# rafaelvp-db/databricks-distributed-deep-learning

Measured on AMD Instinct MI355X. Metric: ResNet-50 images/sec (whole node), higher is better.
Workload: dtype bf16

## Files before the change

### csrc/kernels/gemm_duo.hip

```cpp
#include "ddl_lds.h"

#include <cstdlib>

namespace {

constexpr int TM = 256, TN = 128, DBK = 32, NST = 3, NTH = 256;
constexpr int A_BYTES = TM * DBK * 2;
constexpr int B_BYTES = TN * DBK * 2;
constexpr int ST_BYTES = A_BYTES + B_BYTES;
constexpr int GROUP_M = 8;

enum { LKC = 0, LKO = 1, LCONV = 2 };
enum { E_BF16 = 0, E_GELU = 1, E_DGELU = 2, E_BNB = 3 };

struct DuoParams {
    const bf16_t* A;
    const bf16_t* B;
    long lda, ldb;
    bf16_t* C;
    long ldc;
    int M, N, K;
    const bf16_t* bias;
    const bf16_t* res;
    bf16_t* aux;
    float* colstats;
    int tiles_m, tiles_n;
    int cN, cH, cW, cC, cP, cQ, cstride, h_off, w_off, h_step, w_step, cR, cS;
    FastDiv fd_PQ, fd_Q, fd_C, fd_S;
    const uint8_t* bn_mask;
    const float* bn_mean;
    const float* bn_istd;
    int splits, kt_per_split;
    bf16_t* ws;
    int accumulate;
    const bf16_t* zero;
};

__device__ __forceinline__ bf16x8 frag_kc(const char* sub) {
    const int l = threadIdx.x & 63;
    return *reinterpret_cast<const bf16x8*>(sub + swz_kc((l & 15) * 64 + (l >> 4) * 16));
}
__device__ __attribute__((aligned(16))) uint4 g_duo_zero[1];

template <int LA, int LB, int EK>
__global__ __launch_bounds__(NTH, 2) void gemm_duo_k(DuoParams p) {
    __shared__ __attribute__((aligned(16))) char smem[NST * ST_BYTES];
    const int w = __builtin_amdgcn_readfirstlane(threadIdx.x >> 6), l = threadIdx.x & 63;
    const int wm = w >> 1, wn = w & 1;

    int tm, tn, split = 0;
    {
        const int nwg = p.tiles_m * p.tiles_n, n = nwg * p.splits, bid = blockIdx.x;
        const int xcd = bid & 7, qn = n >> 3, rn = n & 7;
        const int q = (xcd < rn ? xcd * (qn + 1) : rn * (qn + 1) + (xcd - rn) * qn) + (bid >> 3);
        split = q / nwg;
        const int wg = q - split * nwg;
        const int per_group = GROUP_M * p.tiles_n;
        const int grp = wg / per_group, first_m = grp * GROUP_M;
        const int gsz = min(p.tiles_m - first_m, GROUP_M);
        const int wl = wg - grp * per_group;
        tm = first_m + wl % gsz;
        tn = wl / gsz;
    }
    const int m0 = tm * TM, n0 = tn * TN;
    const int kbase = split * p.kt_per_split;
    const int nt = min(p.K / DBK - kbase, p.kt_per_split);

    const int lb = swz_kc(l * 16);
    const int r_in = lb >> 6, kcol = ((lb >> 4) & 3) * 8;
    const long a_bytes = LA == LCONV ? (long)p.cN * p.cH * p.cW * p.cC * 2
                       : (LA == LKO ? (long)p.K * p.lda * 2 : (long)p.M * p.lda * 2);
    const __amdgpu_buffer_rsrc_t ars_op =
        __builtin_amdgcn_make_buffer_rsrc(const_cast<bf16_t*>(p.A), 0, (int)a_bytes, 0x00020000);
    const __amdgpu_buffer_rsrc_t brs_op = __builtin_amdgcn_make_buffer_rsrc(
        const_cast<bf16_t*>(p.B), 0, (int)((long)(LB == LKC ? p.N : p.K) * p.ldb * 2), 0x00020000);
    int ao[4], bo[2];
    const bf16_t* abase[4];
    uint32_t vmask[4];
#pragma unroll
    for (int s = 0; s < 4; ++s) {
        const int m = m0 + (4 * w + s) * 16 + r_in;
        if (LA == LCONV) {
            const int mm = m < p.M ? m : 0;
            const int n = (int)fdiv((uint32_t)mm, p.fd_PQ);
            const int rem = mm - n * p.cP * p.cQ;
            const int pp = (int)fdiv((uint32_t)rem, p.fd_Q);
            const int qq = rem - pp * p.cQ;
            const int hb = pp * p.cstride + p.h_off, wb = qq * p.cstride + p.w_off;
            uint32_t mk = 0;
            if (m < p.M) {
                for (int rr = 0; rr < p.cR; ++rr)
                    for (int ss = 0; ss < p.cS; ++ss) {
                        const int hh = hb + rr * p.h_step, ww = wb + ss * p.w_step;
                        if ((unsigned)hh < (unsigned)p.cH && (unsigned)ww < (unsigned)p.cW) mk |= 1u << (rr * p.cS + ss);
                    }
            }
            vmask[s] = mk;
            abase[s] = p.A + ((long)(n * p.cH + hb) * p.cW + wb) * p.cC + kcol;
            ao[s] = 0;
        } else if (LA == LKO) {
            const int u = 4 * w + s, krow = (u & 7) * 4 + (l >> 4);
            ao[s] = (krow * (int)p.lda + m0 + (u >> 3) * 128 + 8 * ((l & 15) ^ swz_ko(krow))) * 2;
        } else {
            ao[s] = (min(m, p.M - 1) * (int)p.lda + kcol) * 2;
        }
    }
#pragma unroll
    for (int s = 0; s < 2; ++s) {
        if (LB == LKC) {
            bo[s] = ((n0 + (2 * w + s) * 16 + r_in) * (int)p.ldb + kcol) * 2;
        } else {
            const int krow = (2 * w + s) * 4 + (l >> 4);
            bo[s] = (krow * (int)p.ldb + n0 + 8 * ((l & 15) ^ swz_ko(krow))) * 2;
        }
    }
    const int b_kstep = LB == LKC ? DBK * 2 : DBK * (int)p.ldb * 2;
    auto stage = [&](int kt, int slot) {
        kt += kbase;
        char* sb = smem + slot * ST_BYTES;
        if constexpr (LA == LKO) {
#pragma unroll
            for (int s = 0; s < 4; ++s) {
                const int u = 4 * w + s;
                __builtin_amdgcn_raw_ptr_buffer_load_lds(ars_op, (lds_void*)(sb + (u >> 3) * 8192 + (u & 7) * 1024), 16,
                                                         ao[s], kt * DBK * (int)p.lda * 2, 0, 0);
            }
        } else if constexpr (LA == LCONV) {
            const int k0 = kt * DBK;
            const int tap = (int)fdiv((uint32_t)k0, p.fd_C), ci = k0 - tap * p.cC;
            const int rr = (int)fdiv((uint32_t)tap, p.fd_S), ss = tap - rr * p.cS;
            const long toff = (long)(rr * p.h_step * p.cW + ss * p.w_step) * p.cC + ci;
#pragma unroll
            for (int s = 0; s < 4; ++s) {
                const bool ok = (vmask[s] >> tap) & 1u;
                glds16(ok ? abase[s] + toff : p.zero, sb + (4 * w + s) * 1024);
            }
        } else {
#pragma unroll
            for (int s = 0; s < 4; ++s)
                __builtin_amdgcn_raw_ptr_buffer_load_lds(ars_op, (lds_void*)(sb + (4 * w + s) * 1024), 16, ao[s],
                                                         kt * (DBK * 2), 0, 0);
        }
#pragma unroll
        for (int s = 0; s < 2; ++s)
            __builtin_amdgcn_raw_ptr_buffer_load_lds(brs_op, (lds_void*)(sb + A_BYTES + (2 * w + s) * 1024), 16, bo[s],
                                                     kt * b_kstep, 0, 0);
    };

    f32x4 acc[8][4];
#pragma unroll
    for (int i = 0; i < 8; ++i)
#pragma unroll
        for (int j = 0; j < 4; ++j) acc[i][j] = (f32x4){0.f, 0.f, 0.f, 0.f};

    bf16x8 fa0[8], fb0[4], fa1[8], fb1[4];
    auto read_frags = [&](int slot, bf16x8 (&fa)[8], bf16x8 (&fb)[4]) {
        const char* sb = smem + slot * ST_BYTES;
        const int lane = threadIdx.x & 63;
#pragma unroll
        for (int j = 0; j < 4; ++j)
            fb[j] = LB == LKC ? frag_kc(sb + A_BYTES + (wn * 4 + j) * 1024) : frag_ko(sb + A_BYTES, wn * 64 + j * 16, lane);
#pragma unroll
        for (int i = 0; i < 8; ++i) fa[i] = LA == LKO ? frag_ko(sb + wm * 8192, i * 16, lane) : frag_kc(sb + (wm * 8 + i) * 1024);
// ... 33 lines not shown
        const int s1 = slot == 2 ? 0 : slot + 1;
        step(t, slot, fa0, fb0, fa1, fb1);
        step(t + 1, s1, fa1, fb1, fa0, fb0);
        slot = s1 == 2 ? 0 : s1 + 1;
    }
    if (t < nt) step(t, slot, fa0, fb0, fa1, fb1);

    const int r16 = l & 15, g4 = (l >> 4) * 4;
    const int mw = m0 + wm * 128;
    const int nw = n0 + wn * 64;
    const uint32_t cbytes = (uint32_t)((long)p.M * p.ldc * 2);
    float bv[4][4];
#pragma unroll
    for (int j = 0; j < 4; ++j) {
        if (EK != E_DGELU && p.bias) {
            const uint2 b2 = *reinterpret_cast<const uint2*>(p.bias + nw + j * 16 + g4);
            bv[j][0] = lo_f(b2.x); bv[j][1] = hi_f(b2.x); bv[j][2] = lo_f(b2.y); bv[j][3] = hi_f(b2.y);
        } else {
            bv[j][0] = bv[j][1] = bv[j][2] = bv[j][3] = 0.f;
        }
    }
    const bf16_t* pre = EK == E_BF16 ? p.res : (EK == E_DGELU ? (const bf16_t*)p.aux : nullptr);
    float bnm[4][4], bns[4][4];
    if (EK == E_BNB) {
#pragma unroll
        for (int j = 0; j < 4; ++j) {
            const f32x4 mv = *reinterpret_cast<const f32x4*>(p.bn_mean + nw + j * 16 + g4);
            const f32x4 sv = *reinterpret_cast<const f32x4*>(p.bn_istd + nw + j * 16 + g4);
#pragma unroll
            for (int e = 0; e < 4; ++e) { bnm[j][e] = mv[e]; bns[j][e] = sv[e]; }
        }
    }
    u32x2 rb[8][4];
    if (pre) {
        const __amdgpu_buffer_rsrc_t prs =
            __builtin_amdgcn_make_buffer_rsrc(const_cast<bf16_t*>(pre), 0, (int)cbytes, 0x00020000);
#pragma unroll
        for (int i = 0; i < 8; ++i)
#pragma unroll
            for (int j = 0; j < 4; ++j)
                rb[i][j] = __builtin_amdgcn_raw_buffer_load_b64(
                    prs, (int)(((long)(mw + i * 16 + r16) * p.ldc + nw + j * 16 + g4) * 2), 0, 0);
    }
    const int wr0 = wm * 128 + r16;
    auto img_off = [&](int i, int j) {
        const int u = (wn * 8 + j * 2 + (l >> 5)) * 2 + ((l >> 4) & 1);
        return (wr0 + i * 16) * 256 + ((u ^ r16) << 3);
    };
    BARRIER();
    const bool stats = EK != E_GELU && p.colstats;
    u32x2 yk[8][4];
    const __amdgpu_buffer_rsrc_t xrs =
        __builtin_amdgcn_make_buffer_rsrc(EK == E_BNB ? (void*)p.aux : (void*)p.C, 0, (int)cbytes, 0x00020000);
    const __amdgpu_buffer_rsrc_t rrs =
        __builtin_amdgcn_make_buffer_rsrc(EK == E_BNB && p.res ? (void*)p.res : (void*)p.C, 0, (int)cbytes, 0x00020000);
    const __amdgpu_buffer_rsrc_t mrs = __builtin_amdgcn_make_buffer_rsrc(
        EK == E_BNB && p.bn_mask ? (void*)p.bn_mask : (void*)p.C, 0, (int)(cbytes / 16), 0x00020000);
#pragma unroll
    for (int j = 0; j < 4; ++j) {
        float cs[4] = {0.f, 0.f, 0.f, 0.f}, cq[4] = {0.f, 0.f, 0.f, 0.f};
        u32x2 bx[8], br[8];
        uint32_t bmk[8];
        if (EK == E_BNB) {
#pragma unroll
            for (int i = 0; i < 8; ++i) {
                const int o = (mw + i * 16 + r16) * (int)p.ldc + nw + j * 16 + g4;
                bx[i] = __builtin_amdgcn_raw_buffer_load_b64(xrs, o * 2, 0, 0);
                br[i] = p.res ? __builtin_amdgcn_raw_buffer_load_b64(rrs, o * 2, 0, 0) : u32x2{0u, 0u};
                bmk[i] = p.bn_mask ? (uint32_t)__builtin_amdgcn_raw_buffer_load_b8(mrs, o >> 3, 0, 0) >> (o & 4) : 0xfu;
            }
        }
#pragma unroll
        for (int i = 0; i < 8; ++i) {
            const int m = mw + i * 16 + r16;
            const f32x4 a = acc[i][j];
            uint32_t lo, hi;
            if (EK == E_BF16) {
                float rv[4] = {0.f, 0.f, 0.f, 0.f};
                if (pre) { rv[0] = lo_f(rb[i][j][0]); rv[1] = hi_f(rb[i][j][0]); rv[2] = lo_f(rb[i][j][1]); rv[3] = hi_f(rb[i][j][1]); }
                lo = pack2bf(a[0] + bv[j][0] + rv[0], a[1] + bv[j][1] + rv[1]);
                hi = pack2bf(a[2] + bv[j][2] + rv[2], a[3] + bv[j][3] + rv[3]);
                *reinterpret_cast<uint2*>(smem + img_off(i, j)) = make_uint2(lo, hi);
            } else if (EK == E_GELU) {
                const float z[4] = {a[0] + bv[j][0], a[1] + bv[j][1], a[2] + bv[j][2], a[3] + bv[j][3]};
                const f32x2_t y0 = gelu_erf2(f32x2_t{z[0], z[1]}), y1 = gelu_erf2(f32x2_t{z[2], z[3]});
                lo = pack2bf(y0.x, y0.y);
                hi = pack2bf(y1.x, y1.y);
                yk[i][j] = u32x2{lo, hi};
                *reinterpret_cast<uint2*>(smem + img_off(i, j)) =
                    p.aux ? make_uint2(pack2bf(z[0], z[1]), pack2bf(z[2], z[3])) : make_uint2(lo, hi);
            } else if (EK == E_BNB) {
                float v[4];
#pragma unroll
                for (int e = 0; e < 4; ++e) {
                    const uint32_t rw = br[i][e >> 1];
                    const float rv = (e & 1) ? hi_f(rw) : lo_f(rw);
                    v[e] = ((bmk[i] >> e) & 1u) ? a[e] + rv : 0.f;
                }
                lo = pack2bf(v[0], v[1]);
                hi = pack2bf(v[2], v[3]);
                *reinterpret_cast<uint2*>(smem + img_off(i, j)) = make_uint2(lo, hi);
            } else {
                const u32x2 z2 = rb[i][j];
                const f32x2_t d0 = f32x2_t{a[0], a[1]} * gelu_erf_grad2(f32x2_t{lo_f(z2[0]), hi_f(z2[0])});
                const f32x2_t d1 = f32x2_t{a[2], a[3]} * gelu_erf_grad2(f32x2_t{lo_f(z2[1]), hi_f(z2[1])});
                lo = pack2bf(d0.x, d0.y);
                hi = pack2bf(d1.x, d1.y);
                *reinterpret_cast<uint2*>(smem + img_off(i, j)) = make_uint2(lo, hi);
            }
            if (stats) {
                const bool keep = m < p.M;
                const float tv[4] = {keep ? lo_f(lo) : 0.f, keep ? hi_f(lo) : 0.f, keep ? lo_f(hi) : 0.f,
                                     keep ? hi_f(hi) : 0.f};
                if (EK == E_BNB) {
                    const float xv[4] = {lo_f(bx[i][0]), hi_f(bx[i][0]), lo_f(bx[i][1]), hi_f(bx[i][1])};
#pragma unroll
                    for (int e = 0; e < 4; ++e) {
                        cs[e] += tv[e];
                        cq[e] += tv[e] * (xv[e] - bnm[j][e]) * bns[j][e];
                    }
                } else {
#pragma unroll
                    for (int e = 0; e < 4; ++e) {
                        cs[e] += tv[e];
                        cq[e] += tv[e] * tv[e];
                    }
                }
            }
        }
        if (stats) {
#pragma unroll
            for (int e = 0; e < 4; ++e) {
                cs[e] = row16_sum(cs[e]);
                cq[e] = row16_sum(cq[e]);
            }
            if (r16 == 0) {
                float* row = p.colstats + (long)(tm * 2 + wm) * 2 * p.N;
                const int n = nw + j * 16 + g4;
                *reinterpret_cast<f32x4*>(row + n) = (f32x4){cs[0], cs[1], cs[2], cs[3]};
                *reinterpret_cast<f32x4*>(row + p.N + n) = (f32x4){cq[0], cq[1], cq[2], cq[3]};
            }
        }
    }
    auto store_image = [&](bf16_t* dst, long ld, uint32_t bytes, bool acc_c, bool nt = false) {
        asm volatile("s_waitcnt lgkmcnt(0)" ::: "memory");
        BARRIER();
        const __amdgpu_buffer_rsrc_t rs = __builtin_amdgcn_make_buffer_rsrc(dst, 0, (int)bytes, 0x00020000);
        const int c = l & 15;
        const bool odd = (l >> 4) & 1;
#pragma unroll
        for (int it = 0; it < 16; ++it) {
            const int r = w * 64 + it * 4 + (l >> 4);
            u32x4 v = *reinterpret_cast<const u32x4*>(smem + r * 256 + ((c ^ ((r >> 1) & 7)) << 4));
            if (odd) v = u32x4{v[2], v[3], v[0], v[1]};
            const int off = (int)(((long)(m0 + r) * ld + n0 + c * 8) * 2);
            if (acc_c) {
                const u32x4 o = __builtin_amdgcn_raw_buffer_load_b128(rs, off, 0, 0);
#pragma unroll
                for (int e = 0; e < 4; ++e)
                    v[e] = pack2bf(lo_f(v[e]) + lo_f(o[e]), hi_f(v[e]) + hi_f(o[e]));
            }
            if (nt) __builtin_amdgcn_raw_buffer_store_b128(v, rs, off, 0, 2);
            else __builtin_amdgcn_raw_buffer_store_b128(v, rs, off, 0, 0);
        }
    };
    if (p.splits > 1) {
        store_image(p.ws + (long)split * p.M * p.N, p.N, (uint32_t)((long)p.M * p.N * 2), false);
        return;
    }
    if (EK == E_GELU && p.aux) {
        store_image(p.aux, p.ldc, cbytes, false, true);
        asm volatile("s_waitcnt lgkmcnt(0)" ::: "memory");
        BARRIER();
#pragma unroll
        for (int i = 0; i < 8; ++i)
#pragma unroll
            for (int j = 0; j < 4; ++j)
                *reinterpret_cast<uint2*>(smem + img_off(i, j)) = make_uint2(yk[i][j][0], yk[i][j][1]);
    }
    store_image(p.C, p.ldc, cbytes, p.accumulate != 0);
}

__global__ __launch_bounds__(256) void duo_reduce_k(const bf16_t* __restrict__ ws, bf16_t* __restrict__ C, long ldc,
                                                    int M, int N, int splits, int accumulate) {
    const long n8 = N / 8, total = (long)M * n8, slab = (long)M * N;
    for (long i = (long)blockIdx.x * blockDim.x + threadIdx.x; i < total; i += (long)gridDim.x * blockDim.x) {
        const int m = (int)(i / n8), n = (int)(i - (long)m * n8) * 8;
        float v[8] = {0.f, 0.f, 0.f, 0.f, 0.f, 0.f, 0.f, 0.f};
        const bf16_t* pb = ws + (long)m * N + n;
        auto add = [&](const uint4& r) {
            const uint32_t wd[4] = {r.x, r.y, r.z, r.w};
#pragma unroll
            for (int e = 0; e < 4; ++e) { v[2 * e] += lo_f(wd[e]); v[2 * e + 1] += hi_f(wd[e]); }
        };
        int s = 0;
        for (; s + 4 <= splits; s += 4) {
            uint4 r[4];
#pragma unroll
            for (int j = 0; j < 4; ++j) r[j] = *reinterpret_cast<const uint4*>(pb + (s + j) * slab);
#pragma unroll
            for (int j = 0; j < 4; ++j) add(r[j]);
        }
        for (; s < splits; ++s) add(*reinterpret_cast<const uint4*>(pb + s * slab));
        bf16_t* cp = C + (long)m * ldc + n;
        if (accumulate) {
            float o[8];
            load8(cp, o);
#pragma unroll
            for (int e = 0; e < 8; ++e) v[e] += o[e];
        }
        store8(cp, v);
    }
}

template <int LA, int LB>
int launch(const DuoParams& p, int ek, hipStream_t st) {
    const dim3 grid(p.tiles_m * p.tiles_n), block(NTH);
    switch (ek) {
        case E_BF16: hipLaunchKernelGGL((gemm_duo_k<LA, LB, E_BF16>), grid, block, 0, st, p); break;
        case E_GELU: hipLaunchKernelGGL((gemm_duo_k<LA, LB, E_GELU>), grid, block, 0, st, p); break;
        case E_DGELU: hipLaunchKernelGGL((gemm_duo_k<LA, LB, E_DGELU>), grid, block, 0, st, p); break;
        default: hipLaunchKernelGGL((gemm_duo_k<LA, LB, E_BNB>), grid, block, 0, st, p); break;
    }
    return (int)hipGetLastError();
}

}

DDL_API int ddl_gemm_duo(int mode, const void* A, long lda, const void* B, long ldb, void* C, long ldc, int M, int N,
                         int K, const void* bias, int act, void* aux, const void* res, float* colstats, const int* conv,
                         hipStream_t st) {
    BnbArgs bn{};
    if (act == 5) bn = ddl_take_bnb();
    if (M <= 0 || N <= 0) return 0;
    if (mode != 0 && mode != 1 && mode != 3) return -1;
    if (mode == 3 && (!conv || conv[3] % 32 || conv[13] != conv[4] || conv[14] != conv[5] || conv[15] != 1 ||
                      conv[16] != 0 || conv[17] != 0 || K != conv[11] * conv[12] * conv[3] ||
                      conv[11] * conv[12] > 32))
        return -1;
    if (N % TN || K % DBK || K <= 0 || lda % 8 || ldb % 8 || ldc % 8 || (mode != 3 && lda < K) || ldc < N ||
        (mode == 1 ? ldb < N : ldb < K) || ((uintptr_t)A & 15) || ((uintptr_t)B & 15) || ((uintptr_t)C & 15))
        return -1;
    int ek;
    if (act == 0) ek = E_BF16;
    else if (act == 1 && !res) ek = E_GELU;
    else if (act == 4 && aux && !bias && !res) ek = E_DGELU;
    else if (act == 5 && aux && !bias && colstats && bn.mean && bn.istd && ldc == N) ek = E_BNB;
    else return -2;
    if (ek == E_GELU && colstats) return -2;
    if ((res && ((uintptr_t)res & 7)) || (aux && ((uintptr_t)aux & 15)) || (bias && ((uintptr_t)bias & 7))) return -1;
    const long a_bytes = mode == 3 ? (long)conv[0] * conv[1] * conv[2] * conv[3] * 2 : (long)M * lda * 2;
    const long b_bytes = (long)(mode == 1 ? K : N) * ldb * 2, c_bytes = (long)M * ldc * 2;
    if (a_bytes >= (1L << 31) || b_bytes >= (1L << 31) || c_bytes >= (1L << 31)) return -1;
    DuoParams p{};
    p.A = (const bf16_t*)A; p.B = (const bf16_t*)B; p.lda = lda; p.ldb = ldb;
    p.C = (bf16_t*)C; p.ldc = ldc; p.M = M; p.N = N; p.K = K;
    p.bias = (const bf16_t*)bias; p.res = (const bf16_t*)res; p.aux = (bf16_t*)aux; p.colstats = colstats;
    p.bn_mask = bn.mask; p.bn_mean = bn.mean; p.bn_istd = bn.istd;
    p.splits = 1;
    p.kt_per_split = K / DBK;
    p.tiles_m = (M + TM - 1) / TM;
    p.tiles_n = N / TN;
    if (mode == 3) {
        static const bf16_t* zp[64] = {};
        int dev = 0;
        if (hipGetDevice(&dev) != hipSuccess || dev < 0 || dev >= 64) return -1;
        if (!zp[dev]) {
            void* a = nullptr;
            if (hipGetSymbolAddress(&a, HIP_SYMBOL(g_duo_zero)) != hipSuccess || !a) return -1;
            zp[dev] = (const bf16_t*)a;
        }
        p.zero = zp[dev];
        p.cN = conv[0]; p.cH = conv[1]; p.cW = conv[2]; p.cC = conv[3]; p.cP = conv[4]; p.cQ = conv[5];
        p.cstride = conv[6]; p.h_off = conv[7]; p.w_off = conv[8]; p.h_step = conv[9]; p.w_step = conv[10];
        p.cR = conv[11]; p.cS = conv[12];
        p.fd_PQ = make_fastdiv((uint32_t)(p.cP * p.cQ));
        p.fd_Q = make_fastdiv((uint32_t)p.cQ);
        p.fd_C = make_fastdiv((uint32_t)p.cC);
        p.fd_S = make_fastdiv((uint32_t)std::max(1, p.cS));
        return launch<LCONV, LKC>(p, ek, st);
    }
    return mode == 0 ? launch<LKC, LKC>(p, ek, st) : launch<LKC, LKO>(p, ek, st);
}

DDL_API int ddl_gemm_duo_tn(const void* A, long lda, const void* B, long ldb, void* C, long ldc, int M, int N, int K,
                            int splits, int accumulate, void* ws, long ws_elems, hipStream_t st) {
    if (M <= 0 || N <= 0) return 0;
    if (M % TM || N % TN || K % DBK || K <= 0 || lda % 8 || ldb % 8 || ldc % 8 || lda < M || ldb < N || ldc < N ||
        ((uintptr_t)A & 15) || ((uintptr_t)B & 15) || ((uintptr_t)C & 15))
        return -1;
    if ((long)K * lda * 2 >= (1L << 31) || (long)K * ldb * 2 >= (1L << 31) || (long)M * ldc * 2 >= (1L << 31)) return -1;
    const int nkt = K / DBK;
    if (splits < 1) splits = 1;
    if (splits > nkt) splits = nkt;
    DuoParams p{};
    p.A = (const bf16_t*)A; p.B = (const bf16_t*)B; p.lda = lda; p.ldb = ldb;
    p.C = (bf16_t*)C; p.ldc = ldc; p.M = M; p.N = N; p.K = K;
    p.tiles_m = M / TM;
    p.tiles_n = N / TN;
    p.kt_per_split = (nkt + splits - 1) / splits;
    splits = (nkt + p.kt_per_split - 1) / p.kt_per_split;
    p.splits = splits;
    p.accumulate = accumulate;
    if (splits > 1) {
        if (!ws || ws_elems < (long)splits * M * N || ((uintptr_t)ws & 15) || (long)splits * M * N * 2 >= (1L << 31))
            return -1;
        p.ws = (bf16_t*)ws;
    }
    const dim3 grid(p.tiles_m * p.tiles_n * splits);
    hipLaunchKernelGGL((gemm_duo_k<LKO, LKO, E_BF16>), grid, dim3(NTH), 0, st, p);
    if (splits > 1) {
        const long total = (long)M * (N / 8);
        const int g = (int)std::min<long>(16384, (total + 255) / 256);
        duo_reduce_k<<<g, 256, 0, st>>>(p.ws, p.C, ldc, M, N, splits, accumulate);
    }
    const int rc = (int)hipGetLastError();
    return rc ? -rc - 1 : splits;
}
```

### databricks_distributed_deep_learning_amd/ops/_lib.py

```python
from __future__ import annotations

import ctypes
import os
from typing import Optional

import torch

_PKG_DIR = os.path.dirname(os.path.dirname(os.path.abspath(__file__)))
LIB_PATH = os.environ.get("DDL_NATIVE_LIB") or os.path.join(_PKG_DIR, "_native", "libddl_kernels.so")

_lib: Optional[ctypes.CDLL] = None
_load_error: Optional[str] = None
_mode = os.environ.get("DDL_NATIVE", "auto").lower()


class NativeUnavailable(RuntimeError):
    pass


def set_mode(mode: str) -> None:
    global _mode
    if mode not in ("auto", "on", "off"):
        raise ValueError(mode)
    _mode = mode
# ... 79 lines not shown
    "ddl_bn_rows_sum": [P, I, I, P, P, P],
    "ddl_rows_sum_sink": [I, P, I, I, I, P, I, P, P],
    "ddl_bn_stats_partials": [I, P, L, I, P, P],
    "ddl_bn_bwd_partials": [I, P, P, P, P, P, L, I, I, P, P],
    "ddl_bn_bwd_finish": [I, P, P, P, P, P, P, L, L, I, I, P, P, P, P, P, P, P, I, P],
    "ddl_bn_bwd_from_partials": [I, P, I, P, L, P, P, P, P, P, L, I, P, P, P, P, P, I, P],
    "ddl_bn_partials_ws": [I, I],
    "ddl_bn_fwd_train": [I, P, L, I, P, P, P, P, F, F, P, P, P, P, P, P],
    "ddl_bn_eval_coeffs": [I, I, P, P, P, P, F, P, P, P],
    "ddl_bn_apply": [I, P, P, P, P, P, L, I, I, P, P],
    "ddl_bn_apply2": [I, P, P, P, P, P, P, P, L, I, I, P, P],
    "ddl_bn_relu_maxpool": [I, P, P, P, P, P, P, I, I, I, I, I, I, P],
    "ddl_bn_bwd_pool_nblk": [],
    "ddl_bn_bwd_pool": [I, P, P, P, P, P, P, P, I, I, I, I, I, I, P, P, P, P, P, I, P],
    "ddl_bn_bwd_coef_from_partials": [I, P, I, P, L, P, P, L, I, P, P, P, I, P],
    "ddl_bn_bwd_apply_coef": [I, P, P, P, P, P, L, I, P, P],
    "ddl_bn_fwd_from_partials": [I, P, I, L, I, P, P, P, P, F, F, P, P, P, P, P, L],
    "ddl_conv_w_dgrad": [P, P, I, I, I, I, I, I, P, P, P],
    "ddl_conv_w_dgrad_batch": [P, P, I, P],
    "ddl_gelu_bwd_colsum": [I, P, P, P, L, I, P, P, I, I, P],
    "ddl_acc_f32": [I, P, P, L, P],
    "ddl_tanh_bwd": [I, P, P, P, L, P],
    "ddl_copy2d": [I, P, L, L, L, P, L, L, L, P],
    "ddl_add_into": [I, P, P, L, P],
    "ddl_zero": [P, L, P],
    "ddl_rows_add_row": [I, P, P, P, L, L, P],
    "ddl_seq_prepend_add": [I, P, P, P, P, L, L, L, P],
    "ddl_sort_ids_ok": [L, L],
    "ddl_sort_ids": [P, L, P, P, P],
    "ddl_drain_acc": [I, P, P, L, P],
    "ddl_acc_grad": [I, P, P, L, I, I, P],
    "ddl_softmax_topk": [I, P, L, I, I, P, P, P, P],
    "ddl_gemm_conv_multi": [I, I, P, P, P, P, P, L, I, P, P],
    "ddl_conv3x3": [P, P, P, I, I, I, I, I, P, P, P, P, P, P, I, P],
    "ddl_conv3x3_wgrad": [P, P, P, I, I, I, I, I, P, L, I, I, I, P],
    "ddl_stem_wgrad": [P, P, P, I, I, I, I, I, I, I, P, L, I, I, I, P],
    "ddl_stem_fwd": [P, P, P, I, I, I, I, P, I, P],
    "ddl_s2d_input": [P, I, I, I, I, I, P, I, I, P],
    "ddl_s2d_weight": [P, I, I, I, I, P, I, I, P],
    "ddl_skinny_gemm": [P, P, P, L, I, I, P, P, P, P, P, P, I, P],
    "ddl_stream_gemm": [P, P, P, L, I, I, P, P, P, P, P, P, I, P],
    "ddl_stream_wgrad_ws": [I, I],
    "ddl_conv3_bwd_grid": [L, I],
    "ddl_conv3_bwd": [P, P, P, P, P, P, P, P, P, P, P, P, P, P, L, P, I, I, L, I, I, I, P],
    "ddl_bn_bwd": [I, P, P, P, P, P, P, L, I, I, P, P, P, P, P, P, I, P],
    "ddl_ln_supported": [I],
    "ddl_ln_fwd": [I, P, P, L, P, P, P, P, P, L, I, F, U64, F, P],
    "ddl_ln_bwd_nblk": [L],
    "ddl_ln_bwd": [I, P, P, P, L, P, P, P, P, P, P, P, L, I, I, P, U64, F, P, P, P, P],
    "ddl_gelu_fwd": [I, P, P, L, P],
    "ddl_gelu_bwd": [I, P, P, P, L, P],
    "ddl_dropout": [I, P, P, L, U64, F, P],
    "ddl_colsum_nblk": [L],
    "ddl_colsum": [I, P, L, I, P, P, I, I, P],
    "ddl_softmax_ce": [I, P, P, L, I, P, P, P, P],
    "ddl_scale_by": [I, P, P, P, L, P],
    "ddl_maxpool_fwd": [I, P, P, P, I, I, I, I, I, I, I, I, I, P],
    "ddl_maxpool_bwd": [I, P, P, P, I, I, I, I, I, I, I, I, I, P],
    "ddl_avgpool_fwd": [I, P, P, I, I, I, P],
    "ddl_avgpool_bwd": [I, P, P, I, I, I, P],
    "ddl_embedding_fwd": [I, P, P, P, L, I, P],
    "ddl_embedding_bwd": [I, P, P, P, P, L, L, I, I, P],
    "ddl_embedding_bwd_sorted": [I, P, P, P, P, P, L, I, I, P],
    "ddl_sgd_step": [I, P, P, I, P, P, P, I, P, F, F, F, I, I, P],
    "ddl_adamw_step": [I, P, P, I, P, P, P, P, I, P, F, F, F, F, F, F, F, F, F, P],
    "ddl_lamb_step": [I, P, P, I, P, P, P, P, I, P, F, F, F, F, F, F, F, F, F, P, P],
# ... 96 lines not shown
```

### databricks_distributed_deep_learning_amd/ops/_native_conv.py

```python
from __future__ import annotations

import ctypes
import os

import torch
import torch.nn.functional as F

from . import _lib
from ._lib import grad_ready, grad_sink
from ._native_gemm import MODE_CONV, MODE_CONVW, MODE_NN, MODE_NT, MODE_TN, gemm, plan, stats_rows_max
from ._native_norm import _BN_BWD_EPI, _BN_BWD_EPI_RES


def _desc(N, H, W, C, P, Q, stride, h_off, w_off, h_step, w_step, R, S, OH, OW, ostep=1, oa=0, ob=0):
    return [N, H, W, C, P, Q, stride, h_off, w_off, h_step, w_step, R, S, OH, OW, ostep, oa, ob]


STATS_MIN_K = int(os.environ.get("DDL_BN_STATS_MIN_K", "0"))
_DGRAD_NT = os.environ.get("DDL_DGRAD_NT", "1") != "0"


_CONV3X3 = os.environ.get("DDL_CONV3X3", "1") != "0"


# ... 273 lines not shown
            Ho = (H - a + stride - 1) // stride
            Wo = (W_ - b + stride - 1) // stride
            if not rs or not ss or Ho <= 0 or Wo <= 0:
                empty = True
                continue
            classes.append((a, b, rs, ss, Ho, Wo))
    if residual is not None:
        dx = residual if residual.is_contiguous() else residual.contiguous()
    else:
        dx = (torch.zeros if empty else torch.empty)(N, H, W_, C, dtype=dy.dtype, device=dy.device)
    probs = []
    for a, b, rs, ss, Ho, Wo in classes:
        wc = _w_dgrad(w, rs, ss, param)
        h_off = (a + pad - rs[0]) // stride
        w_off = (b + pad - ss[0]) // stride
        Rp, Sp = len(rs), len(ss)
        probs.append((wc, N * Ho * Wo, Rp * Sp * K,
                      _desc(N, P, Q, K, Ho, Wo, 1, h_off, w_off, -1, -1, Rp, Sp, H, W_, stride, a, b)))

    def serial(out, res=None):
        for wc, Mc, Kc, desc in probs:
            gemm(MODE_CONV, dy, 0, wc, Kc, out, C, Mc, C, Kc, conv=desc, row_remap=True, residual=res)

    def multi(out, narrow):
        bs = (ctypes.c_void_p * len(probs))(*[pr[0].data_ptr() for pr in probs])
        ms = (ctypes.c_int * len(probs))(*[pr[1] for pr in probs])
        ks = (ctypes.c_int * len(probs))(*[pr[2] for pr in probs])
        cv = (ctypes.c_int * (18 * len(probs)))(*[v for pr in probs for v in pr[3]])
        rc = _lib.fn("ddl_gemm_conv_multi")(int(narrow), len(probs), dy.data_ptr(), bs, ms, ks, out.data_ptr(), C, C,
                                            cv, _lib.stream())
        if rc != 0:
            raise RuntimeError(f"ddl_gemm_conv_multi failed: {rc}")

    if residual is not None:
        serial(dx, dx)
    elif 1 < len(probs) <= 4:
        key = (tuple(dy.shape), tuple(w.shape), stride, pad)
        choice = _MULTI_CHOICE.get(key)
        if choice is None:
            from . import _native_gemm as NG
            skey = "dgrad_path|" + "|".join(str(v) for v in key)
            planned = NG.lookup_choice(skey)
            if planned is not None and planned[0] in ("serial", "multi", "multi_narrow"):
                choice = _MULTI_CHOICE[key] = planned[0]
            else:
                choice = _pick_dgrad_path(key, serial, multi, dx)
                NG.record_choice(skey, (choice, 1))
        if choice == "serial":
            serial(dx)
        else:
            multi(dx, choice == "multi_narrow")
    else:
        serial(dx)
    return dx


_MULTI_CHOICE: dict = {}


def _pick_dgrad_path(key, serial, multi, dx):
    if not dx.is_cuda or torch.cuda.is_current_stream_capturing():
        return "serial"
    scratch = torch.empty_like(dx)
    serial(scratch)
    cands = {"serial": lambda: serial(scratch), "multi": lambda: multi(scratch, False),
             "multi_narrow": lambda: multi(scratch, True)}
    best, best_t = "serial", float("inf")
    for name, fn in cands.items():
        fn()
        e0, e1 = torch.cuda.Event(enable_timing=True), torch.cuda.Event(enable_timing=True)
        e0.record()
        for _ in range(5):
            fn()
        e1.record()
        e1.synchronize()
        t = e0.elapsed_time(e1)
        if t < best_t:
            best, best_t = name, t
    _MULTI_CHOICE[key] = best
    return best


def _direct3x3_wgrad(dy, x, dw, accumulate, grid=0):
    N, H, W_, C = x.shape
    if (tuple(dy.shape) != (N, H, W_, 64) or tuple(dw.shape) != (64, 3, 3, 64) or not dy.is_contiguous()
            or not x.is_contiguous() or not dw.is_contiguous() or dy.dtype != torch.bfloat16
            or x.dtype != torch.bfloat16 or dw.dtype not in (torch.bfloat16, torch.float32)):
        raise ValueError("direct 3x3 wgrad: operand shapes / layouts not covered")
    g = grid if grid > 0 else 256
    ws = torch.empty(g * 576 * 64, dtype=torch.float32, device=x.device)
    rc = _lib.fn("ddl_conv3x3_wgrad")(x.data_ptr(), dy.data_ptr(), dw.data_ptr(), N, H, W_, C, 64, ws.data_ptr(),
                                      ws.numel(), int(accumulate), int(dw.dtype == torch.float32), int(grid),
                                      _lib.stream())
    if rc != 0:
        raise RuntimeError(f"ddl_conv3x3_wgrad failed: {rc}")
    return dw


def _wgrad(dy, x, w_shape, stride, pad, out=None):
    N, H, W_, C = x.shape
    K, R, S, _ = w_shape
    _, P, Q, _ = dy.shape
    acc = out is not None
    dw = out if acc else torch.empty(K, R, S, C, dtype=dy.dtype, device=dy.device)
    if x.is_cuda and _direct3x3_ok(x.shape, w_shape, stride, pad) and dw.is_contiguous():
        return _direct3x3_wgrad(dy, x, dw, acc)
    M = N * P * Q
    if R == 1 and S == 1 and stride == 1 and pad == 0:
        gemm(MODE_TN, dy, K, x, C, dw, C, K, C, M, accumulate=acc)
    else:
        gemm(MODE_CONVW, dy, K, x, 0, dw, R * S * C, K, R * S * C, M, accumulate=acc,
             conv=_desc(N, H, W_, C, P, Q, stride, -pad, -pad, 1, 1, R, S, P, Q))
    return dw
# ... 315 lines not shown
```

Measured before the change: 12960.

## Add multi-class duo GEMM kernel for strided conv dgrad with fused BN-backward epilogue

```diff
diff --git a/csrc/kernels/gemm_duo.hip b/csrc/kernels/gemm_duo.hip
--- a/csrc/kernels/gemm_duo.hip
+++ b/csrc/kernels/gemm_duo.hip
@@ -1,5 +1,7 @@
 #include "ddl_lds.h"
 
+#include <algorithm>
+#include <climits>
 #include <cstdlib>
 
 namespace {
@@ -12,6 +14,16 @@
 
 enum { LKC = 0, LKO = 1, LCONV = 2 };
 enum { E_BF16 = 0, E_GELU = 1, E_DGELU = 2, E_BNB = 3 };
+
+constexpr int MAX_CLS = 4;
+struct DuoClass {
+    const bf16_t* B;
+    int M, K, tiles_m;
+    int tile0;
+    int prow0;
+    int cP, cQ, h_off, w_off, cR, cS, oa, ob;
+    FastDiv fd_PQ, fd_Q, fd_S;
+};
 
 struct DuoParams {
     const bf16_t* A;
@@ -34,7 +46,12 @@
     bf16_t* ws;
     int accumulate;
     const bf16_t* zero;
+    int OH, OW, ostep;
+    DuoClass cls[MAX_CLS];
 };
+
+constexpr int ROW_NONE = 0x3ff00000;
+constexpr int ROWTAB = TM * 256;
 
 __device__ __forceinline__ bf16x8 frag_kc(const char* sub) {
     const int l = threadIdx.x & 63;
@@ -42,29 +59,60 @@
 }
 __device__ __attribute__((aligned(16))) uint4 g_duo_zero[1];
 
-template <int LA, int LB, int EK>
+template <int LA, int LB, int EK, bool MC = false>
 __global__ __launch_bounds__(NTH, 2) void gemm_duo_k(DuoParams p) {
     __shared__ __attribute__((aligned(16))) char smem[NST * ST_BYTES];
     const int w = __builtin_amdgcn_readfirstlane(threadIdx.x >> 6), l = threadIdx.x & 63;
     const int wm = w >> 1, wn = w & 1;
 
     int tm, tn, split = 0;
+    const int kcls = MC ? (int)(blockIdx.x >= (unsigned)p.cls[1].tile0) + (int)(blockIdx.x >= (unsigned)p.cls[2].tile0) +
+                            (int)(blockIdx.x >= (unsigned)p.cls[3].tile0)
+                      : 0;
+#define DUO_PICK(f) (kcls == 0 ? p.cls[0].f : (kcls == 1 ? p.cls[1].f : (kcls == 2 ? p.cls[2].f : p.cls[3].f)))
+    const bf16_t* const mc_B = MC ? DUO_PICK(B) : nullptr;
+    const int mc_M = MC ? DUO_PICK(M) : 0, mc_K = MC ? DUO_PICK(K) : 0;
+    const int mc_tiles_m = MC ? DUO_PICK(tiles_m) : 0, mc_prow0 = MC ? DUO_PICK(prow0) : 0;
+    const int mc_cP = MC ? DUO_PICK(cP) : 0, mc_cQ = MC ? DUO_PICK(cQ) : 0;
+    const int mc_h_off = MC ? DUO_PICK(h_off) : 0, mc_w_off = MC ? DUO_PICK(w_off) : 0;
+    const int mc_cR = MC ? DUO_PICK(cR) : 0, mc_cS = MC ? DUO_PICK(cS) : 0;
+    const int oa = MC ? DUO_PICK(oa) : 0, ob = MC ? DUO_PICK(ob) : 0;
+    const FastDiv mc_fd_PQ = MC ? FastDiv{DUO_PICK(fd_PQ.d), DUO_PICK(fd_PQ.mul), DUO_PICK(fd_PQ.shift)} : FastDiv{};
+    const FastDiv mc_fd_Q = MC ? FastDiv{DUO_PICK(fd_Q.d), DUO_PICK(fd_Q.mul), DUO_PICK(fd_Q.shift)} : FastDiv{};
+    const FastDiv mc_fd_S = MC ? FastDiv{DUO_PICK(fd_S.d), DUO_PICK(fd_S.mul), DUO_PICK(fd_S.shift)} : FastDiv{};
+#define pB (MC ? mc_B : p.B)
+#define pM (MC ? mc_M : p.M)
+#define pK (MC ? mc_K : p.K)
+#define pldb (MC ? (long)mc_K : p.ldb)
+#define ptiles_m (MC ? mc_tiles_m : p.tiles_m)
+#define prow0 mc_prow0
+#define cP (MC ? mc_cP : p.cP)
+#define cQ (MC ? mc_cQ : p.cQ)
+#define h_off (MC ? mc_h_off : p.h_off)
+#define w_off (MC ? mc_w_off : p.w_off)
+#define cR (MC ? mc_cR : p.cR)
+#define cS (MC ? mc_cS : p.cS)
+#define fd_PQ (MC ? mc_fd_PQ : p.fd_PQ)
+#define fd_Q (MC ? mc_fd_Q : p.fd_Q)
+#define fd_S (MC ? mc_fd_S : p.fd_S)
     {
-        const int nwg = p.tiles_m * p.tiles_n, n = nwg * p.splits, bid = blockIdx.x;
+        const int nwg = ptiles_m * p.tiles_n, n = nwg * (MC ? 1 : p.splits);
+        const int bid = MC ? (int)blockIdx.x - DUO_PICK(tile0) : (int)blockIdx.x;
+#undef DUO_PICK
         const int xcd = bid & 7, qn = n >> 3, rn = n & 7;
         const int q = (xcd < rn ? xcd * (qn + 1) : rn * (qn + 1) + (xcd - rn) * qn) + (bid >> 3);
         split = q / nwg;
         const int wg = q - split * nwg;
         const int per_group = GROUP_M * p.tiles_n;
         const int grp = wg / per_group, first_m = grp * GROUP_M;
-        const int gsz = min(p.tiles_m - first_m, GROUP_M);
+        const int gsz = min(ptiles_m - first_m, GROUP_M);
         const int wl = wg - grp * per_group;
         tm = first_m + wl % gsz;
         tn = wl / gsz;
     }
     const int m0 = tm * TM, n0 = tn * TN;
     const int kbase = split * p.kt_per_split;
-    const int nt = min(p.K / DBK - kbase, p.kt_per_split);
+    const int nt = MC ? pK / DBK : min(p.K / DBK - kbase, p.kt_per_split);
 
     const int lb = swz_kc(l * 16);
     const int r_in = lb >> 6, kcol = ((lb >> 4) & 3) * 8;
@@ -73,7 +121,7 @@
     const __amdgpu_buffer_rsrc_t ars_op =
         __builtin_amdgcn_make_buffer_rsrc(const_cast<bf16_t*>(p.A), 0, (int)a_bytes, 0x00020000);
     const __amdgpu_buffer_rsrc_t brs_op = __builtin_amdgcn_make_buffer_rsrc(
-        const_cast<bf16_t*>(p.B), 0, (int)((long)(LB == LKC ? p.N : p.K) * p.ldb * 2), 0x00020000);
+        const_cast<bf16_t*>(pB), 0, (int)((long)(LB == LKC ? p.N : p.K) * pldb * 2), 0x00020000);
     int ao[4], bo[2];
     const bf16_t* abase[4];
     uint32_t vmask[4];
@@ -81,18 +129,18 @@
     for (int s = 0; s < 4; ++s) {
         const int m = m0 + (4 * w + s) * 16 + r_in;
         if (LA == LCONV) {
-            const int mm = m < p.M ? m : 0;
-            const int n = (int)fdiv((uint32_t)mm, p.fd_PQ);
-            const int rem = mm - n * p.cP * p.cQ;
-            const int pp = (int)fdiv((uint32_t)rem, p.fd_Q);
-            const int qq = rem - pp * p.cQ;
-            const int hb = pp * p.cstride + p.h_off, wb = qq * p.cstride + p.w_off;
+            const int mm = m < pM ? m : 0;
+            const int n = (int)fdiv((uint32_t)mm, fd_PQ);
+            const int rem = mm - n * cP * cQ;
+            const int pp = (int)fdiv((uint32_t)rem, fd_Q);
+            const int qq = rem - pp * cQ;
+            const int hb = pp * p.cstride + h_off, wb = qq * p.cstride + w_off;
             uint32_t mk = 0;
-            if (m < p.M) {
-                for (int rr = 0; rr < p.cR; ++rr)
-                    for (int ss = 0; ss < p.cS; ++ss) {
+            if (m < pM) {
+                for (int rr = 0; rr < cR; ++rr)
+                    for (int ss = 0; ss < cS; ++ss) {
                         const int hh = hb + rr * p.h_step, ww = wb + ss * p.w_step;
-                        if ((unsigned)hh < (unsigned)p.cH && (unsigned)ww < (unsigned)p.cW) mk |= 1u << (rr * p.cS + ss);
+                        if ((unsigned)hh < (unsigned)p.cH && (unsigned)ww < (unsigned)p.cW) mk |= 1u << (rr * cS + ss);
                     }
             }
             vmask[s] = mk;
@@ -102,19 +150,19 @@
             const int u = 4 * w + s, krow = (u & 7) * 4 + (l >> 4);
             ao[s] = (krow * (int)p.lda + m0 + (u >> 3) * 128 + 8 * ((l & 15) ^ swz_ko(krow))) * 2;
         } else {
-            ao[s] = (min(m, p.M - 1) * (int)p.lda + kcol) * 2;
+            ao[s] = (min(m, pM - 1) * (int)p.lda + kcol) * 2;
         }
     }
 #pragma unroll
     for (int s = 0; s < 2; ++s) {
         if (LB == LKC) {
-            bo[s] = ((n0 + (2 * w + s) * 16 + r_in) * (int)p.ldb + kcol) * 2;
+            bo[s] = ((n0 + (2 * w + s) * 16 + r_in) * (int)pldb + kcol) * 2;
         } else {
             const int krow = (2 * w + s) * 4 + (l >> 4);
-            bo[s] = (krow * (int)p.ldb + n0 + 8 * ((l & 15) ^ swz_ko(krow))) * 2;
-        }
-    }
-    const int b_kstep = LB == LKC ? DBK * 2 : DBK * (int)p.ldb * 2;
+            bo[s] = (krow * (int)pldb + n0 + 8 * ((l & 15) ^ swz_ko(krow))) * 2;
+        }
+    }
+    const int b_kstep = LB == LKC ? DBK * 2 : DBK * (int)pldb * 2;
     auto stage = [&](int kt, int slot) {
         kt += kbase;
         char* sb = smem + slot * ST_BYTES;
@@ -128,7 +176,7 @@
         } else if constexpr (LA == LCONV) {
             const int k0 = kt * DBK;
             const int tap = (int)fdiv((uint32_t)k0, p.fd_C), ci = k0 - tap * p.cC;
-            const int rr = (int)fdiv((uint32_t)tap, p.fd_S), ss = tap - rr * p.cS;
+            const int rr = (int)fdiv((uint32_t)tap, fd_S), ss = tap - rr * cS;
             const long toff = (long)(rr * p.h_step * p.cW + ss * p.w_step) * p.cC + ci;
 #pragma unroll
             for (int s = 0; s < 4; ++s) {
@@ -228,7 +276,7 @@
         }
     }
     u32x2 rb[8][4];
-    if (pre) {
+    if (!MC && pre) {
         const __amdgpu_buffer_rsrc_t prs =
             __builtin_amdgcn_make_buffer_rsrc(const_cast<bf16_t*>(pre), 0, (int)cbytes, 0x00020000);
 #pragma unroll
@@ -244,6 +292,33 @@
         return (wr0 + i * 16) * 256 + ((u ^ r16) << 3);
     };
     BARRIER();
+    int rowel[8];
+    if constexpr (MC) {
+        const int m = m0 + (int)threadIdx.x;
+        int off = ROW_NONE;
+        if (m < pM) {
+            const int n = (int)fdiv((uint32_t)m, fd_PQ);
+            const int rem = m - n * cP * cQ;
+            const int pp = (int)fdiv((uint32_t)rem, fd_Q);
+            const int qq = rem - pp * cQ;
+            off = ((n * p.OH + pp * p.ostep + oa) * p.OW + qq * p.ostep + ob) * (int)p.ldc;
+        }
+        *reinterpret_cast<int*>(smem + ROWTAB + (int)threadIdx.x * 4) = off;
+        asm volatile("s_waitcnt lgkmcnt(0)" ::: "memory");
+        BARRIER();
+#pragma unroll
+        for (int i = 0; i < 8; ++i)
+            rowel[i] = *reinterpret_cast<const int*>(smem + ROWTAB + (wm * 128 + i * 16 + r16) * 4);
+        if (pre) {
+            const __amdgpu_buffer_rsrc_t prs =
+                __builtin_amdgcn_make_buffer_rsrc(const_cast<bf16_t*>(pre), 0, (int)cbytes, 0x00020000);
+#pragma unroll
+            for (int i = 0; i < 8; ++i)
+#pragma unroll
+                for (int j = 0; j < 4; ++j)
+                    rb[i][j] = __builtin_amdgcn_raw_buffer_load_b64(prs, (rowel[i] + nw + j * 16 + g4) * 2, 0, 0);
+        }
+    }
     const bool stats = EK != E_GELU && p.colstats;
     u32x2 yk[8][4];
     const __amdgpu_buffer_rsrc_t xrs =
@@ -260,7 +335,7 @@
         if (EK == E_BNB) {
 #pragma unroll
             for (int i = 0; i < 8; ++i) {
-                const int o = (mw + i * 16 + r16) * (int)p.ldc + nw + j * 16 + g4;
+                const int o = (MC ? rowel[i] : (mw + i * 16 + r16) * (int)p.ldc) + nw + j * 16 + g4;
                 bx[i] = __builtin_amdgcn_raw_buffer_load_b64(xrs, o * 2, 0, 0);
                 br[i] = p.res ? __builtin_amdgcn_raw_buffer_load_b64(rrs, o * 2, 0, 0) : u32x2{0u, 0u};
                 bmk[i] = p.bn_mask ? (uint32_t)__builtin_amdgcn_raw_buffer_load_b8(mrs, o >> 3, 0, 0) >> (o & 4) : 0xfu;
@@ -305,7 +380,7 @@
                 *reinterpret_cast<uint2*>(smem + img_off(i, j)) = make_uint2(lo, hi);
             }
             if (stats) {
-                const bool keep = m < p.M;
+                const bool keep = m < pM;
                 const float tv[4] = {keep ? lo_f(lo) : 0.f, keep ? hi_f(lo) : 0.f, keep ? lo_f(hi) : 0.f,
                                      keep ? hi_f(hi) : 0.f};
                 if (EK == E_BNB) {
@@ -331,7 +406,7 @@
                 cq[e] = row16_sum(cq[e]);
             }
             if (r16 == 0) {
-                float* row = p.colstats + (long)(tm * 2 + wm) * 2 * p.N;
+                float* row = p.colstats + (long)(prow0 + tm * 2 + wm) * 2 * p.N;
                 const int n = nw + j * 16 + g4;
                 *reinterpret_cast<f32x4*>(row + n) = (f32x4){cs[0], cs[1], cs[2], cs[3]};
                 *reinterpret_cast<f32x4*>(row + p.N + n) = (f32x4){cq[0], cq[1], cq[2], cq[3]};
@@ -349,7 +424,8 @@
             const int r = w * 64 + it * 4 + (l >> 4);
             u32x4 v = *reinterpret_cast<const u32x4*>(smem + r * 256 + ((c ^ ((r >> 1) & 7)) << 4));
             if (odd) v = u32x4{v[2], v[3], v[0], v[1]};
-            const int off = (int)(((long)(m0 + r) * ld + n0 + c * 8) * 2);
+            const int off = MC ? (*reinterpret_cast<const int*>(smem + ROWTAB + r * 4) + n0 + c * 8) * 2
+                               : (int)(((long)(m0 + r) * ld + n0 + c * 8) * 2);
             if (acc_c) {
                 const u32x4 o = __builtin_amdgcn_raw_buffer_load_b128(rs, off, 0, 0);
 #pragma unroll
@@ -376,6 +452,22 @@
     }
     store_image(p.C, p.ldc, cbytes, p.accumulate != 0);
 }
+
+#undef pB
+#undef pM
+#undef pK
+#undef pldb
+#undef ptiles_m
+#undef prow0
+#undef cP
+#undef cQ
+#undef h_off
+#undef w_off
+#undef cR
+#undef cS
+#undef fd_PQ
+#undef fd_Q
+#undef fd_S
 
 __global__ __launch_bounds__(256) void duo_reduce_k(const bf16_t* __restrict__ ws, bf16_t* __restrict__ C, long ldc,
                                                     int M, int N, int splits, int accumulate) {
@@ -419,6 +511,18 @@
         default: hipLaunchKernelGGL((gemm_duo_k<LA, LB, E_BNB>), grid, block, 0, st, p); break;
     }
     return (int)hipGetLastError();
+}
+
+const bf16_t* duo_zero_page() {
+    static const bf16_t* zp[64] = {};
+    int dev = 0;
+    if (hipGetDevice(&dev) != hipSuccess || dev < 0 || dev >= 64) return nullptr;
+    if (!zp[dev]) {
+        void* a = nullptr;
+        if (hipGetSymbolAddress(&a, HIP_SYMBOL(g_duo_zero)) != hipSuccess || !a) return nullptr;
+        zp[dev] = (const bf16_t*)a;
+    }
+    return zp[dev];
 }
 
 }
@@ -458,15 +562,8 @@
     p.tiles_m = (M + TM - 1) / TM;
     p.tiles_n = N / TN;
     if (mode == 3) {
-        static const bf16_t* zp[64] = {};
-        int dev = 0;
-        if (hipGetDevice(&dev) != hipSuccess || dev < 0 || dev >= 64) return -1;
-        if (!zp[dev]) {
-            void* a = nullptr;
-            if (hipGetSymbolAddress(&a, HIP_SYMBOL(g_duo_zero)) != hipSuccess || !a) return -1;
-            zp[dev] = (const bf16_t*)a;
-        }
-        p.zero = zp[dev];
+        p.zero = duo_zero_page();
+        if (!p.zero) return -1;
         p.cN = conv[0]; p.cH = conv[1]; p.cW = conv[2]; p.cC = conv[3]; p.cP = conv[4]; p.cQ = conv[5];
         p.cstride = conv[6]; p.h_off = conv[7]; p.w_off = conv[8]; p.h_step = conv[9]; p.w_step = conv[10];
         p.cR = conv[11]; p.cS = conv[12];
@@ -513,3 +610,72 @@
     const int rc = (int)hipGetLastError();
     return rc ? -rc - 1 : splits;
 }
+
+DDL_API int ddl_gemm_duo_conv_multi(int n, const void* A, const void* const* Bs, const int* Ms, const int* Ks, void* C,
+                                    long ldc, int N, const int* convs, int act, const void* aux, const void* res,
+                                    float* colstats, hipStream_t st) {
+    BnbArgs bn{};
+    if (act == 5) bn = ddl_take_bnb();
+    if (n < 2 || n > MAX_CLS || !A || !Bs || !Ms || !Ks || !C || !convs) return -1;
+    if (act != 0 && act != 5) return -2;
+    if (act == 5 && !(aux && colstats && bn.mean && bn.istd && ldc == N)) return -2;
+    const int* c0 = convs;
+    const int cN = c0[0], cH = c0[1], cW = c0[2], cC = c0[3], OH = c0[13], OW = c0[14], ostep = c0[15];
+    if (cN <= 0 || cH <= 0 || cW <= 0 || cC <= 0 || cC % DBK || OH <= 0 || OW <= 0 || ostep < 1 || n != ostep * ostep)
+        return -1;
+    if (N <= 0 || N % TN || ldc % 8 || ldc < N || ((uintptr_t)A & 15) || ((uintptr_t)C & 15) ||
+        (res && ((uintptr_t)res & 7)) || (aux && ((uintptr_t)aux & 15)))
+        return -1;
+    const long a_bytes = (long)cN * cH * cW * cC * 2, rows = (long)cN * OH * OW, c_bytes = rows * ldc * 2;
+    if (a_bytes >= (1L << 31) || c_bytes > (1L << 30)) return -1;
+    int order[MAX_CLS];
+    for (int i = 0; i < n; ++i) order[i] = i;
+    std::stable_sort(order, order + n, [&](int a, int b) { return Ks[a] > Ks[b]; });
+    DuoParams p{};
+    p.A = (const bf16_t*)A; p.C = (bf16_t*)C; p.ldc = ldc; p.M = (int)rows; p.N = N;
+    p.res = (const bf16_t*)res; p.aux = (bf16_t*)const_cast<void*>(aux); p.colstats = act == 5 ? colstats : nullptr;
+    p.bn_mask = bn.mask; p.bn_mean = bn.mean; p.bn_istd = bn.istd;
+    p.splits = 1;
+    p.tiles_n = N / TN;
+    p.cN = cN; p.cH = cH; p.cW = cW; p.cC = cC; p.cstride = 1; p.h_step = c0[9]; p.w_step = c0[10];
+    p.fd_C = make_fastdiv((uint32_t)cC);
+    p.OH = OH; p.OW = OW; p.ostep = ostep;
+    long sum_m = 0;
+    int tiles = 0, prow = 0;
+    unsigned seen = 0;
+    for (int k = 0; k < MAX_CLS; ++k) {
+        DuoClass& c = p.cls[k];
+        if (k >= n) { c.tile0 = INT_MAX; continue; }
+        const int i = order[k];
+        const int* d = convs + 18 * i;
+        const int P = d[4], Q = d[5], R = d[11], S = d[12], oa = d[16], ob = d[17];
+        if (d[0] != cN || d[1] != cH || d[2] != cW || d[3] != cC || d[6] != 1 || d[9] != p.h_step || d[10] != p.w_step ||
+            d[13] != OH || d[14] != OW || d[15] != ostep)
+            return -1;
+        if (P <= 0 || Q <= 0 || R <= 0 || S <= 0 || R * S > 32 || oa < 0 || oa >= ostep || ob < 0 || ob >= ostep ||
+            (P - 1) * ostep + oa >= OH || (Q - 1) * ostep + ob >= OW || (seen >> (oa * ostep + ob)) & 1u)
+            return -1;
+        seen |= 1u << (oa * ostep + ob);
+        if (Ms[i] != cN * P * Q || Ks[i] != R * S * cC || !Bs[i] || ((uintptr_t)Bs[i] & 15) ||
+            (long)N * Ks[i] * 2 >= (1L << 31))
+            return -1;
+        c.B = (const bf16_t*)Bs[i]; c.M = Ms[i]; c.K = Ks[i];
+        c.tiles_m = (c.M + TM - 1) / TM;
+        c.tile0 = tiles; c.prow0 = prow;
+        c.cP = P; c.cQ = Q; c.h_off = d[7]; c.w_off = d[8]; c.cR = R; c.cS = S; c.oa = oa; c.ob = ob;
+        c.fd_PQ = make_fastdiv((uint32_t)(P * Q));
+        c.fd_Q = make_fastdiv((uint32_t)Q);
+        c.fd_S = make_fastdiv((uint32_t)S);
+        tiles += c.tiles_m * p.tiles_n;
+        prow += 2 * c.tiles_m;
+        sum_m += c.M;
+    }
+    if (sum_m != rows) return -1;
+    p.zero = duo_zero_page();
+    if (!p.zero) return -1;
+    const dim3 grid(tiles), block(NTH);
+    if (act == 5) hipLaunchKernelGGL((gemm_duo_k<LCONV, LKC, E_BNB, true>), grid, block, 0, st, p);
+    else hipLaunchKernelGGL((gemm_duo_k<LCONV, LKC, E_BF16, true>), grid, block, 0, st, p);
+    const int rc = (int)hipGetLastError();
+    return rc ? -rc - 2 : (act == 5 ? prow : 0);
+}
diff --git a/databricks_distributed_deep_learning_amd/ops/_lib.py b/databricks_distributed_deep_learning_amd/ops/_lib.py
--- a/databricks_distributed_deep_learning_amd/ops/_lib.py
+++ b/databricks_distributed_deep_learning_amd/ops/_lib.py
@@ -135,6 +135,7 @@
     "ddl_acc_grad": [I, P, P, L, I, I, P],
     "ddl_softmax_topk": [I, P, L, I, I, P, P, P, P],
     "ddl_gemm_conv_multi": [I, I, P, P, P, P, P, L, I, P, P],
+    "ddl_gemm_duo_conv_multi": [I, P, P, P, P, P, L, I, P, I, P, P, P, P],
     "ddl_conv3x3": [P, P, P, I, I, I, I, I, P, P, P, P, P, P, I, P],
     "ddl_conv3x3_wgrad": [P, P, P, I, I, I, I, I, P, L, I, I, I, P],
     "ddl_stem_wgrad": [P, P, P, I, I, I, I, I, I, I, P, L, I, I, I, P],
diff --git a/databricks_distributed_deep_learning_amd/ops/_native_conv.py b/databricks_distributed_deep_learning_amd/ops/_native_conv.py
--- a/databricks_distributed_deep_learning_amd/ops/_native_conv.py
+++ b/databricks_distributed_deep_learning_amd/ops/_native_conv.py
@@ -329,40 +329,87 @@
         if rc != 0:
             raise RuntimeError(f"ddl_gemm_conv_multi failed: {rc}")
 
+    def duo(out, res=None, hint=None, part=None):
+        bs = (ctypes.c_void_p * len(probs))(*[pr[0].data_ptr() for pr in probs])
+        ms = (ctypes.c_int * len(probs))(*[pr[1] for pr in probs])
+        ks = (ctypes.c_int * len(probs))(*[pr[2] for pr in probs])
+        cv = (ctypes.c_int * (18 * len(probs)))(*[v for pr in probs for v in pr[3]])
+        if hint is not None:
+            _lib.fn("ddl_gemm_bnb")(_lib.p(hint.mask), _lib.p(hint.mean), _lib.p(hint.istd))
+        rc = _lib.fn("ddl_gemm_duo_conv_multi")(len(probs), dy.data_ptr(), bs, ms, ks, out.data_ptr(), C, C, cv,
+                                                5 if hint is not None else 0,
+                                                hint.x.data_ptr() if hint is not None else 0, _lib.p(res),
+                                                _lib.p(part), _lib.stream())
+        if rc < 0:
+            raise RuntimeError(f"ddl_gemm_duo_conv_multi failed: {rc}")
+        return rc
+
+    duo_ok = (dy.is_cuda and dy.dtype == torch.bfloat16 and w.dtype == torch.bfloat16 and not empty
+              and 1 < len(probs) <= 4 and len(probs) == stride * stride and C % 128 == 0 and K % 32 == 0
+              and R * S <= 32 and dy.numel() * 2 < 2 ** 31 and N * H * W_ * C * 2 <= 2 ** 30
+              and dy.data_ptr() % 16 == 0 and dx.data_ptr() % 16 == 0)
+    choice = None
+    if duo_ok or (residual is None and 1 < len(probs) <= 4):
+        choice = _dgrad_choice((tuple(dy.shape), tuple(w.shape), stride, pad), serial, multi,
+                               duo if duo_ok else None, dx)
+    if choice == "duo" and duo_ok:
+        out = torch.empty_like(dx) if residual is not None else dx
+        hint = bnb if (bnb is not None and bnb.x.is_contiguous() and bnb.x.data_ptr() % 16 == 0
+                       and (bnb.mask is None or bnb.mask.numel() * 8 >= dx.numel())) else None
+        if hint is not None:
+            rows = 2 * sum(-(-pr[1] // 256) for pr in probs)
+            part = torch.empty((rows + -(-rows // 32)) * 2 * C, dtype=torch.float32, device=dx.device)
+            hint.set(out, part, duo(out, residual, hint, part))
+        else:
+            duo(out, residual)
+        return out
     if residual is not None:
         serial(dx, dx)
-    elif 1 < len(probs) <= 4:
-        key = (tuple(dy.shape), tuple(w.shape), stride, pad)
-        choice = _MULTI_CHOICE.get(key)
-        if choice is None:
-            from . import _native_gemm as NG
-            skey = "dgrad_path|" + "|".join(str(v) for v in key)
-            planned = NG.lookup_choice(skey)
-            if planned is not None and planned[0] in ("serial", "multi", "multi_narrow"):
-                choice = _MULTI_CHOICE[key] = planned[0]
-            else:
-                choice = _pick_dgrad_path(key, serial, multi, dx)
-                NG.record_choice(skey, (choice, 1))
-        if choice == "serial":
-            serial(dx)
-        else:
-            multi(dx, choice == "multi_narrow")
+    elif choice in ("multi", "multi_narrow"):
+        multi(dx, choice == "multi_narrow")
     else:
         serial(dx)
     return dx
 
 
 _MULTI_CHOICE: dict = {}
-
-
-def _pick_dgrad_path(key, serial, multi, dx):
+_DGRAD_PATHS = ("serial", "multi", "multi_narrow")
+
+
+def _dgrad_choice(key, serial, multi, duo, dx):
+    choice = _MULTI_CHOICE.get(key)
+    if choice is not None:
+        return choice
+    from . import _native_gemm as NG
+    tail = "|".join(str(v) for v in key)
+    planned = NG.lookup_choice("dgrad_path|" + tail)
+    path = planned[0] if planned is not None and planned[0] in _DGRAD_PATHS else None
+    on = None
+    if duo is not None:
+        planned = NG.lookup_choice("dgrad_duo|" + tail)
+        on = None if planned is None else planned[0] == "duo"
+    if path is None or (duo is not None and on is None):
+        best, best_path = _pick_dgrad_path(key, serial, multi, dx, duo)
+        if path is None:
+            path = best_path
+            NG.record_choice("dgrad_path|" + tail, (path, 1))
+        if duo is not None and on is None:
+            on = best == "duo"
+            NG.record_choice("dgrad_duo|" + tail, ("duo" if on else "small", 1))
+    choice = _MULTI_CHOICE[key] = "duo" if on else path
+    return choice
+
+
+def _pick_dgrad_path(key, serial, multi, dx, duo=None):
     if not dx.is_cuda or torch.cuda.is_current_stream_capturing():
-        return "serial"
+        return "serial", "serial"
     scratch = torch.empty_like(dx)
     serial(scratch)
     cands = {"serial": lambda: serial(scratch), "multi": lambda: multi(scratch, False),
              "multi_narrow": lambda: multi(scratch, True)}
-    best, best_t = "serial", float("inf")
+    if duo is not None:
+        cands["duo"] = lambda: duo(scratch)
+    times = {}
     for name, fn in cands.items():
         fn()
         e0, e1 = torch.cuda.Event(enable_timing=True), torch.cuda.Event(enable_timing=True)
@@ -371,11 +418,9 @@
             fn()
         e1.record()
         e1.synchronize()
-        t = e0.elapsed_time(e1)
-        if t < best_t:
-            best, best_t = name, t
-    _MULTI_CHOICE[key] = best
-    return best
+        times[name] = e0.elapsed_time(e1)
+    best = min(times, key=times.get)
+    return best, min(_DGRAD_PATHS, key=times.get)
 
 
 def _direct3x3_wgrad(dy, x, dw, accumulate, grid=0):
```

Result: no change. 13030, median of 6 (+0.5%).
